# TAMUCrypto/virgo-plus

Measured on AMD Instinct MI355X. Metric: prover sec + field-ops/sec, SHA-256 circuit, 1/2/4/8 MI355X (bit-exact), higher is better.
Workload: dtype u64 (F_p^2, p=2^61-1); 1 GPU; SHA-256 1024-block circuit (SHA256_64.pws x1024, 102347776 gates, 15 layers, 2^23 input wires), GKR sumcheck + Virgo FFT/LDT commit on GPU (BASELINE configs[2]); pass_mode=sync, field_ops_per_proof=8299342697

## Files before the change

include/vpgpu.h:

```cpp
#ifndef VPGPU_H
#define VPGPU_H
#include <stdint.h>
#ifdef __cplusplus
extern "C" {
#endif

typedef struct vp_ctx vp_ctx;
typedef struct { uint64_t real, img; } vp_F;

enum {
    VP_OK = 0,
    VP_EINVAL = -1,
    VP_EHIP = -2,
    VP_ENOGPU = -3,
    VP_EASSERT = -4,
    VP_ELIMIT = -5,
    VP_EXCHANGE = 1
};

enum { VP_MUL = 0, VP_ADD, VP_SUB, VP_ANTISUB, VP_NAAB, VP_ANTINAAB, VP_INPUT, VP_MULC, VP_ADDC, VP_XOR, VP_NOT, VP_COPY };

typedef struct {
    uint64_t size;
    int32_t bit_length;
// ... 13 lines not shown
typedef struct {
    uint32_t struct_size;
    uint32_t abi;
    int32_t use_graph;
    int32_t plan_autotune;
    int32_t real_values;
    int32_t real_pairs;
    int32_t pc_tensor_pub;
    int32_t persistent_rounds;
    int32_t persistent_timeout_ms;
    int32_t poll;
    int32_t prefetch_round1;
    int32_t interactive_fast_init;
    int32_t split_cost_percent;
    int32_t debug;
    int32_t reserved[4];
} vp_options;
void vp_options_default(vp_options *opt);

int vp_create(int device, vp_ctx **out);
int vp_create_with_options(int device, const vp_options *opt, vp_ctx **out);
int vp_get_options(const vp_ctx *, vp_options *out);
int vp_tuning_get(const vp_ctx *, const char *name, int32_t *value);
int vp_test_drivers(void);
int vp_plan_tuning_get(const vp_ctx *, int32_t v[6]);
int vp_plan_tuning_set(vp_ctx *, const int32_t v[6]);
#define VP_WARM_COMMITMENT 1u
#define VP_WARM_FFT_GKR 2u
int vp_warm(vp_ctx *, uint32_t what);
void vp_destroy(vp_ctx *);
const char *vp_last_error(const vp_ctx *);
const char *vp_version(void);
int vp_checked_build(void);

int vp_circuit_upload(vp_ctx *, int n_layers, const vp_layer_desc *layers);

int vp_evaluate(vp_ctx *, const vp_F *inputs, uint64_t n_inputs);
int vp_layer_values(vp_ctx *, int layer, vp_F *out, uint64_t n);

int vp_vres(vp_ctx *, const vp_F *r_0, int r_0_size, vp_F *out);

int vp_phase1_init(vp_ctx *, int layer, const vp_F *r_liu, const vp_F *assert_random);
int vp_phase2_init(vp_ctx *, int layer, const vp_F *r_u);
int vp_liu_init(vp_ctx *, int layer, const vp_F *r_u, const vp_F *const *r_v, const vp_F *s);

int vp_round(vp_ctx *, const vp_F *previous_random, vp_F out_poly[3]);
// ... 94 lines not shown
int vp_get_resident_resumes(const vp_ctx *, uint64_t *n);
int vp_set_profiling(vp_ctx *, int level);

enum { VP_K_BETA = 0, VP_K_LIGHT, VP_K_CHUNKS, VP_K_COMBINE, VP_K_DOT, VP_K_DOTFIN, VP_K_SFGEN, VP_K_SF, VP_K_SEG, VP_K_EMIT,
       VP_K_FIXUP, VP_K_NTT_SPLIT, VP_K_NTT_LDS, VP_K_NTT_UNSPLIT, VP_K_LEAF_HASH, VP_K_MERKLE, VP_K_PC_POINTWISE, VP_K_FRI_FOLD,
       VP_K_ROUND, VP_K_NTT8_COLS, VP_K_NTT8_ROWS, VP_K_NTT_LONG_SPLIT, VP_K_NTT_LONG_MERGE, VP_K_PC_POLY_EVAL, VP_K_PC_POLY_EVAL_FIN, VP_K_PC_OPENING_DIGESTS,
       VP_K_PC_OPEN_MANY, VP_K_COUNT };
typedef struct {
    int32_t kind;
    int32_t step;
    uint32_t workgroups;
    uint32_t jobs;
    uint32_t rounds, first_round;
    uint64_t bytes;
    uint64_t work;
    double us;
} vp_launch_stat;
int vp_get_launch_stats(vp_ctx *, vp_launch_stat *out, int capacity, int *n);
const char *vp_kernel_name(int kind);

int vp_test_field(vp_ctx *, int op, const vp_F *a, const vp_F *b, vp_F *out, uint64_t n);
int vp_test_beta(vp_ctx *, const vp_F *r, int n, const vp_F *init, vp_F *out);
int vp_test_sha3(vp_ctx *, const uint8_t *in, uint8_t *out, uint64_t n);
int vp_test_fft(vp_ctx *, const vp_F *coefs, int coef_len, int order, int inverse, vp_F *out);
int vp_test_fs_draw(vp_ctx *, int op, const uint8_t state[32], const uint8_t root[32], uint64_t label, uint64_t counter, uint8_t state_out[32], vp_F *r_out);

#ifdef __cplusplus
}
#endif
#endif
```

virgo-plus_amd/__init__.py:

```python
import ctypes
import os
import shutil
import subprocess

PKG_DIR = os.path.dirname(os.path.abspath(__file__))
ROOT = os.path.dirname(PKG_DIR)
CSRC = os.path.join(PKG_DIR, "csrc")
HOST = os.path.join(PKG_DIR, "host")
LIB_GPU = os.environ.get("VP_LIBGPU") or os.path.join(CSRC, "libvpgpu.so")
LIB_GPU_CHECKED = os.path.join(ROOT, "tools", "_build", "checked", "libvpgpu.so")
LIB_GPU_TESTDRV = os.path.join(ROOT, "tools", "_build", "testdrv", "libvpgpu.so")
LIB_HOST = os.path.join(HOST, "libvphost.so")
CLI = os.path.join(HOST, "virgo_plus_run")

GPU_SRC = [os.path.join(CSRC, f) for f in ("vpgpu.hip", "vpgpu_batched.inc", "vpgpu_pc.inc", "vpgpu_pc_shard.inc", "vpgpu_pcverify.inc", "vp_kernels_pcverify.h", "vpgpu_fftgkr.inc", "vpgpu_gkrfs.inc", "vpgpu_upload.inc", "vp_kernels_fftgkr.h", "vp_kernels_gkrfs.h", "vp_kernels.h", "vp_kernels_round.h", "vp_kernels_persist.h", "vp_kernels_batch.h",
                                              "vp_kernels_plan.h", "vp_kernels_pc.h", "vp_kernels_ntt8.h", "vp_kernels_ntt_long.h", "vp_keccak_asm.h", "vp_check.h", "vp_field.h", "vp_fri_layout.h", "vp_pc_live.h", "vp_pc_corners.h")] + [
    os.path.join(ROOT, "include", "vpgpu.h")]
HOST_SRC = [os.path.join(HOST, f) for f in ("circuit.cpp", "prover.cpp", "verifier.cpp", "vphost.cpp")]
HOST_HDR = [os.path.join(HOST, f) for f in ("circuit.hpp", "prover.hpp", "verifier.hpp", "vphost.h", "field.hpp",
                                              "polynomial.hpp", "sha3.hpp", "pc_fs.hpp", "fft_gkr_fs.hpp", "gkr_fs.hpp", "fft_gkr_verify.hpp")]


def _stale(target, sources):
    if not os.path.exists(target):
# ... 65 lines not shown

_gpu = None
_host = None


def lib_gpu():
    global _gpu
    if _gpu is None:
        if not os.path.exists(LIB_GPU):
            raise RuntimeError("libvpgpu.so is not built: run __graft_entry__.build()")
        L = ctypes.CDLL(LIB_GPU, mode=ctypes.RTLD_GLOBAL)
        vp = ctypes.c_void_p
        L.vp_create.argtypes = [ctypes.c_int, ctypes.POINTER(vp)]
        L.vp_create_with_options.argtypes = [ctypes.c_int, vp, ctypes.POINTER(vp)]
        L.vp_get_options.argtypes = [vp, vp]
        L.vp_get_resident_resumes.argtypes = [vp, ctypes.POINTER(ctypes.c_uint64)]
        L.vp_set_shard_split.argtypes = [vp, ctypes.c_int]
        L.vp_set_round_shard.argtypes = [vp, ctypes.c_int, ctypes.c_int, ctypes.c_int]
        L.vp_get_round_shard.argtypes = [vp, ctypes.POINTER(ctypes.c_int), ctypes.POINTER(ctypes.c_int), ctypes.POINTER(ctypes.c_int)]
        L.vp_shard_finish.argtypes = [vp, vp, ctypes.c_uint64, vp]
        L.vp_gkr_sizes.argtypes = [vp, vp, vp]
        L.vp_options_default.argtypes = [vp]
        L.vp_tuning_get.argtypes = [vp, ctypes.c_char_p, ctypes.POINTER(ctypes.c_int32)]
        u64_ = ctypes.c_uint64
        L.vp_set_deferred.argtypes = [vp, ctypes.c_int]
        L.vp_warm.argtypes = [vp, ctypes.c_uint32]
        L.vp_flush.argtypes = [vp, ctypes.c_int]
        L.vp_pending.argtypes = [vp, ctypes.POINTER(ctypes.c_int)]
        L.vp_pc_hash_late.argtypes = [vp, ctypes.c_int]
        L.vp_phase_ms.argtypes = [vp, ctypes.POINTER(ctypes.c_double)]
        L.vp_commit_private.argtypes = [vp, vp]
        L.vp_fft_gkr_sizes.argtypes = [ctypes.c_int, vp, vp]
        L.vp_fft_gkr.argtypes = [vp, ctypes.c_int, vp, u64_, vp, u64_, vp]
        L.vp_fft_gkr_begin.argtypes = [vp, ctypes.c_int, vp, u64_]
        L.vp_fft_gkr_end.argtypes = [vp, vp, u64_, vp]
        L.vp_fft_gkr_cancel.argtypes = [vp]
        L.vp_fft_gkr_fs.argtypes = [vp, ctypes.c_int, vp, vp, u64_, vp, vp, vp]
        L.vp_options_default.restype = None
        L.vp_destroy.argtypes = [vp]
        L.vp_last_error.argtypes = [vp]
        L.vp_last_error.restype = ctypes.c_char_p
        L.vp_version.restype = ctypes.c_char_p
        L.vp_test_field.argtypes = [vp, ctypes.c_int, vp, vp, vp, ctypes.c_uint64]
        L.vp_test_beta.argtypes = [vp, vp, ctypes.c_int, vp, vp]
        L.vp_test_sha3.argtypes = [vp, vp, vp, ctypes.c_uint64]
        L.vp_test_fft.argtypes = [vp, vp, ctypes.c_int, ctypes.c_int, ctypes.c_int, vp]
# ... 649 lines not shown
        nd = ctypes.c_uint64(0)
        if lib_host().vph_gkr_fs_tape(self.h, ctypes.cast(st_in, ctypes.c_void_p), ctypes.cast(buf, ctypes.c_void_p), len(transcript), tape.ctypes.data, ctypes.byref(nd),
                                      ctypes.cast(st_out, ctypes.c_void_p)):
            raise ValueError("gkr_fs_tape: malformed transcript")
        return tape, int(nd.value), st_out.raw

    def verify_fs(self, proof):
        buf = ctypes.create_string_buffer(bytes(proof), len(proof))
        return lib_host().vph_verify_fs(self.h, ctypes.cast(buf, ctypes.c_void_p), len(proof)) == 0

    def close(self):
        if self.h:
            lib_host().vph_circuit_free(self.h)
            self.h = None


_PUBLIC_OPTIONS = ("use_graph", "plan_autotune", "real_values", "real_pairs", "pc_tensor_pub", "persistent_rounds", "persistent_timeout_ms", "poll", "prefetch_round1",
                   "interactive_fast_init", "split_cost_percent", "debug")
_TUNING_ENV = {"gkr_path": "VP_GKR_PATH", "serial": "VP_GKR_SERIAL", "fuse_init": "VP_FUSE_INIT", "fuse_min_log": "VP_FUSE_MIN_LOG", "fuse_dot": "VP_FUSE_DOT",
               "drop_y": "VP_DROP_Y", "drop_y_round1": "VP_DROP_Y1", "seg_tiny": "VP_SEG_TINY", "sf_big_log": "VP_SF_BIG_LOG", "sf3b_grid": "VP_SF3B_GRID",
               "dot_blocks": "VP_DOT_BLOCKS", "plan_align": "VP_PLAN_ALIGN", "round_fused_max": "VP_ROUND_FUSED_MAX",
               "kernel_copies": "VP_KERNEL_COPIES", "fold_branches": "VP_FOLD_BRANCHES", "fuse_combine": "VP_FUSE_COMBINE",
               "graph_explicit": "VP_GRAPH_EXPLICIT", "ntt_r8": "VP_NTT_R8", "fuse_p2": "VP_FUSE_P2", "leaf_asm": "VP_LEAF_ASM",
               "fft_gkr_batched": "VP_FFT_GKR_BATCHED", "split_vu": "VP_SPLIT_VU", "pc_live": "VP_PC_LIVE"}
VP_OPTIONS_ABI = 0x76700005


class Options(ctypes.Structure):
    _fields_ = [("struct_size", ctypes.c_uint32), ("abi", ctypes.c_uint32)] + [(n, ctypes.c_int32) for n in _PUBLIC_OPTIONS] + [("reserved", ctypes.c_int32 * 4)]

    def __init__(self, **kw):
        super().__init__()
        lib_gpu().vp_options_default(ctypes.byref(self))
        self.tuning = {}
        for k, v in kw.items():
            if k in _PUBLIC_OPTIONS:
                setattr(self, k, v)
            elif k in _TUNING_ENV:
                self.tuning[k] = v
            else:
                raise TypeError("unknown option " + k)

    def tuning_env(self):
        env = {}
        for k, v in getattr(self, "tuning", {}).items():
            if k == "gkr_path":
                v = {PATH_PLAN: "plan", PATH_LANES: "lanes", PATH_SIMPLE: "simple"}[v]
# ... 599 lines not shown
```

virgo-plus_amd/csrc/vp_kernels_pc.h:

```cpp
#pragma once
#include "vp_kernels_round.h"
#include "vp_keccak_asm.h"
#define f_mul f_mul_plain

namespace vp {

__device__ __forceinline__ F root_raw(const F *__restrict__ RT, u32 half_m , u32 e ) { return RT[e & (half_m - 1)]; }
__device__ __forceinline__ F root_fin(const F &r, u32 half_m, u32 e) {
    const bool neg = e >= half_m;
    const u64 nre = r.re ? P61 - r.re : 0, nim = r.im ? P61 - r.im : 0;
    return f_make(neg ? nre : r.re, neg ? nim : r.im);
}
__device__ __forceinline__ F root_pow(const F *__restrict__ RT, u32 half_m, u32 e) { return root_fin(root_raw(RT, half_m, e), half_m, e); }
__device__ __forceinline__ void loads_first() { __builtin_amdgcn_sched_barrier(0); }
__global__ void __launch_bounds__(VP_BLOCK)
k_root_table_step(F *RT, u32 have , F step ) {
    u32 i = blockIdx.x * blockDim.x + threadIdx.x;
    if (i < have) RT[have + i] = f_mul(RT[i], step);
}
__global__ void __launch_bounds__(VP_BLOCK) k_root_compact(const F *__restrict__ RT, u32 stride, u32 n, F *__restrict__ out) {
    const u32 k = blockIdx.x * blockDim.x + threadIdx.x;
    if (k < n) out[k] = RT[(size_t) k * stride];
}

// ... 252 lines not shown
__global__ void __launch_bounds__(VP_BLOCK) k_merkle_top_fs(MerkleArgs a, Dig *roots, Dig *state, u64 label, u64 counter, F *r_next) {
    merkle_top_body(a, roots);
    if (blockIdx.x == 0 && threadIdx.x == 0) fs_absorb_draw(state, a.tree[0] + 1, label, counter, r_next);
}
__global__ void k_fs_draw(Dig *state, const Dig *root, u64 label, u64 counter, F *r_out) {
    if (blockIdx.x == 0 && threadIdx.x == 0) fs_absorb_draw(state, root, label, counter, r_out);
}
__global__ void k_test_fs_limbs(const u64 *__restrict__ in, u64 *__restrict__ out, u32 n) {
    const u32 i = blockIdx.x * blockDim.x + threadIdx.x;
    if (i < n) out[i] = fs_limb(in[i]);
}

#ifdef VP_LEAF_STAMPS
__device__ unsigned long long g_leaf_stamps[4 * 65536];
__device__ unsigned int g_leaf_stamp_n;
#define VP_LEAF_STAMP_BEGIN const u64 st_t0 = __builtin_amdgcn_s_memtime(), st_r0 = __builtin_amdgcn_s_memrealtime();
#define VP_LEAF_STAMP_END(tag) if (threadIdx.x == 0) { const u64 st_t1 = __builtin_amdgcn_s_memtime(), st_r1 = __builtin_amdgcn_s_memrealtime(); \
        const u32 sl = atomicAdd(&g_leaf_stamp_n, 1u) & 65535u; g_leaf_stamps[4 * sl] = st_t0; g_leaf_stamps[4 * sl + 1] = st_r0; g_leaf_stamps[4 * sl + 2] = st_t1; \
        g_leaf_stamps[4 * sl + 3] = (st_r1 << 1) | (tag); }
#else
#define VP_LEAF_STAMP_BEGIN
#define VP_LEAF_STAMP_END(tag)
#endif
template <bool MASK> __global__ void __launch_bounds__(VP_LEAF_ASM_THREADS) k_leaf_hash(FriLeafArgs a) {
    VP_LEAF_STAMP_BEGIN
    const u32 total = a.leaf_start[a.n];
    const u32 g = blockIdx.x * blockDim.x + threadIdx.x, gc = g < total ? g : total - 1;
    int j = 0;
    while (j + 1 < a.n && gc >= a.leaf_start[j + 1]) ++j;
    const u32 t = gc - a.leaf_start[j], N = a.N[j];
    const F *cw = a.cw[j];
    const bool last = N == 1;
    const u32 halfN = last ? 16u : N >> 1;
    const u32 p = last ? t : t % halfN, b = last ? 0u : t / halfN;
    const F *x = cw + (size_t) b * N + p;
    if constexpr (MASK) {
        const F *m = a.mask[j] + (size_t) b * N + p;
        vp_leaf_chain_mask_asm(x, x + halfN, 32u * N * 16u, 64u, m, m + halfN, a.leaves[j] + (last ? t : 32 * p + b), g < total ? 1u : 0u);
    } else
        vp_leaf_chain_asm(x, x + halfN, 32u * N * 16u, 64u, a.leaves[j] + (last ? t : 32 * p + b), g < total ? 1u : 0u);
    VP_LEAF_STAMP_END(a.n > 1 ? 1u : 0u)
}

__global__ void k_test_sha3(const u64 *__restrict__ in, u64 *__restrict__ out, u32 n) {
    u32 i = blockIdx.x * blockDim.x + threadIdx.x;
    if (i >= n) return;
    Dig h; h.w[0] = in[8 * i + 4]; h.w[1] = in[8 * i + 5]; h.w[2] = in[8 * i + 6]; h.w[3] = in[8 * i + 7];
    Dig d = hhash64(in[8 * i], in[8 * i + 1], in[8 * i + 2], in[8 * i + 3], h);
    out[4 * i] = d.w[0]; out[4 * i + 1] = d.w[1]; out[4 * i + 2] = d.w[2]; out[4 * i + 3] = d.w[3];
}

}

namespace vp {

__global__ void __launch_bounds__(VP_BLOCK)
k_pc_products(const F *__restrict__ lcw, const F *__restrict__ qcw, u32 N, F *__restrict__ P, u32 n_slices, const F *__restrict__ q0,
              const F *__restrict__ qscal) {
    const u32 t = blockIdx.x * blockDim.x + threadIdx.x;
    if (t >= 2 * n_slices * N) return;
    const u32 a = t % N, r = t / N, i = r >> 1, b = (r & 1) ? 16 : 0;
    const size_t src = ((size_t) i * 32 + b) * N + a;
    const F q = q0 ? f_mul(qscal[i], q0[(size_t) b * N + a]) : qcw[src];
    P[t] = f_mul(lcw[src], q);
// ... 485 lines not shown
```

virgo-plus_amd/csrc/vpgpu.hip:

```cpp
#include <hip/hip_runtime.h>

#include <algorithm>
#include <chrono>
#include <cstdio>
#include <cstring>
#include <deque>
#include <functional>
#include <map>
#include <mutex>
#include <set>
#include <atomic>
#include <string>
#include <thread>
#include <vector>

#include "../../include/vpgpu.h"
#include "vp_kernels.h"
#include "vp_fri_layout.h"
#include "vp_pc_live.h"
#include "vp_pc_corners.h"

using namespace vp;

static_assert(sizeof(vp_F) == sizeof(F), "vp_F layout");
// ... 107 lines not shown
    int32_t drop_y;
    int32_t drop_y_round1;
    int32_t real_values;
    int32_t seg_tiny;
    int32_t sf_big_log;
    int32_t sf3b_grid;
    int32_t dot_blocks;
    int32_t plan_align;
    int32_t round_fused_max;
    int32_t persistent_rounds, poll, debug, prefetch_round1, split_cost_percent;
    int32_t kernel_copies;
    int32_t fold_branches;
    int32_t fuse_combine;
    int32_t plan_autotune, pc_tensor_pub, persistent_timeout_ms;
    int32_t graph_explicit;
    int32_t ntt_r8;
    int32_t interactive_fast_init;
    int32_t fuse_p2;
    int32_t leaf_asm;
    int32_t real_pairs;
    int32_t fft_gkr_batched;
    int32_t split_vu;
    int32_t pc_live;
};

struct vp_ctx {
    int device = 0;
    hipStream_t stream = nullptr;
    std::string err = "";
    int n_layers = 0, max_bl = 0;
    std::vector<LayerDev> L;
    F **d_vals = nullptr;
    unsigned long long **d_valsr = nullptr;
    F *beta_g = nullptr, *beta_u = nullptr, *bf = nullptr, *bs = nullptr, *liu_half = nullptr;
    u32 half_cap = 0;
    F *tab[2][3] = {{nullptr, nullptr, nullptr}, {nullptr, nullptr, nullptr}};
    u32 cap = 0;
    F *partials = nullptr;
    unsigned int *round_arrivals = nullptr;
    F *small = nullptr;
    F *chunk_part = nullptr; u32 chunk_cap = 0;
    F *d_tape = nullptr; u64 n_tape = 0;
    F *d_tr = nullptr; u64 n_tr = 0;
    F *h_pin = nullptr;
    unsigned long long *h_seq = nullptr, seq = 0;
    TailMail *h_req = nullptr; TailReply *h_rep = nullptr; std::atomic<bool> tail_active{false}; unsigned long long tail_seq = 0; int tail_enabled = 1;
// ... 51 lines not shown
    int hash_late = 0;
    unsigned pc_unhashed = 0;
    uint8_t *late_root[2] = {nullptr, nullptr};

    PcShard *pcs = nullptr;
    FgkState *fgk = nullptr;
    VpComm *cm = nullptr;
    F *part2 = nullptr;
    int simple_path = 0, serial = 0;
    Lane lane0; Lane *ln = nullptr;
    std::vector<Lane> lanes;
    std::vector<hipStream_t> lane_streams; std::vector<hipEvent_t> lane_events; hipEvent_t ev_fork = nullptr;
    F *pred_r = nullptr, *pred_pool = nullptr, *pred_part = nullptr, *pred_out = nullptr; BetaJob *pred_jobs = nullptr; u32 pred_bpj = 1;
    DotJob *pred_dot = nullptr; BlkMap *pred_map = nullptr;
    PlanRec *rec = nullptr;
    DotJob rec_dot{};
    SfGenJob rec_gen{};
    int fuse_init = 1;
    Plan *plan = nullptr; int plan_path = 1;
    std::recursive_mutex mu;
    bool plan_tuned = false;
    bool plan_tune_cached = false;
    int leaf_attr_done = 0;
    uint32_t opt_pinned = 0;
    hipGraphExec_t gkr_graph = nullptr; int use_graph = 1; bool graph_failed = false; u64 graph_launches = 0, graph_rounds = 0;
    int shard_rank = 0, shard_world = 1;
    int split_lw = 0, split_min_log = 11;
    struct SplitTab { int j, bl; u32 slot0; };
    struct SplitChain { u64 poly_pos = 0, claims_pos = 0, r_off = 0; int rounds = 0, has_a = 1, n_tab = 0, small_owner = 0; std::vector<SplitTab> tabs; };
    std::vector<SplitChain> split;
    F *d_trs = nullptr; u64 n_exp = 0;
    F *tr_base() const { return (split_lw > 0 && d_trs) ? d_trs : d_tr; }
    std::vector<int> chain_owner;
    std::vector<double> chain_cost;
    bool drop_round1 = false;
    std::vector<FixJob> rec_fix;
    bool owned(int chain) const { return shard_world <= 1 || chain_owner.empty() || chain_owner[chain] == shard_rank; }
    bool vu_supplied = false; float vu_pre_ms = 0; u64 vu_tape_tag = 0;
    RoundShard *rsh = nullptr;
    bool sc_open = false;

    F *zero() const { return small; }
    F *one() const { return small + 1; }
    F *add_term() const { return small + 2; }
    F *Vu() const { return small + 3; }
    F *coef() const { return small + 4; }
// ... 667 lines not shown
    return 0;
#endif
}
const char *vp_version(void) { return "vpgpu 0.1 (gfx950)"; }
const char *vp_last_error(const vp_ctx *ctx) { return ctx ? ctx->err.c_str() : "null context"; }

static void opt_defaults(VpOpt *o) {
    memset(o, 0, sizeof *o);
    o->gkr_path = VP_PATH_PLAN; o->use_graph = 1; o->serial = 0; o->fuse_init = 1; o->fuse_min_log = 0; o->fuse_dot = 0;
    o->drop_y = 1; o->drop_y_round1 = 0; o->real_values = 1; o->seg_tiny = 1; o->sf_big_log = 14;
    o->sf3b_grid = 512; o->dot_blocks = 1024; o->plan_align = 0; o->round_fused_max = 512;
    o->persistent_rounds = 1; o->poll = 1; o->debug = 0; o->prefetch_round1 = 1; o->split_cost_percent = 50; o->kernel_copies = 1; o->fold_branches = 1; o->fuse_combine = 2; o->plan_autotune = 1;
    o->pc_tensor_pub = 1;
    o->persistent_timeout_ms = 10000;
    o->graph_explicit = 0;
    o->ntt_r8 = 1;
    o->interactive_fast_init = 1;
    o->fuse_p2 = 1;
    o->leaf_asm = 1;
    o->real_pairs = 1;
    o->fft_gkr_batched = 1;
    o->split_vu = 1;
    o->pc_live = 1;
}
static void opt_to_public(const VpOpt &o, vp_options *p) {
    memset(p, 0, sizeof *p);
    p->struct_size = (uint32_t) sizeof *p; p->abi = VP_OPTIONS_ABI;
    p->use_graph = o.use_graph; p->plan_autotune = o.plan_autotune; p->real_values = o.real_values; p->real_pairs = o.real_pairs; p->pc_tensor_pub = o.pc_tensor_pub;
    p->persistent_rounds = o.persistent_rounds; p->persistent_timeout_ms = o.persistent_timeout_ms; p->poll = o.poll; p->prefetch_round1 = o.prefetch_round1;
    p->interactive_fast_init = o.interactive_fast_init; p->split_cost_percent = o.split_cost_percent; p->debug = o.debug;
}
void vp_options_default(vp_options *p) {
    if (!p) return;
    VpOpt o; opt_defaults(&o);
    opt_to_public(o, p);
}
int vp_test_drivers(void) {
#ifdef VP_TEST_DRIVERS
    return 1;
#else
    return 0;
#endif
}
struct OptName { const char *name; int32_t VpOpt::*field; };
static const OptName g_opt_names[] = {
    {"gkr_path", &VpOpt::gkr_path}, {"use_graph", &VpOpt::use_graph}, {"serial", &VpOpt::serial}, {"fuse_init", &VpOpt::fuse_init}, {"fuse_min_log", &VpOpt::fuse_min_log},
    {"fuse_dot", &VpOpt::fuse_dot}, {"drop_y", &VpOpt::drop_y}, {"drop_y_round1", &VpOpt::drop_y_round1}, {"real_values", &VpOpt::real_values}, {"seg_tiny", &VpOpt::seg_tiny},
    {"sf_big_log", &VpOpt::sf_big_log}, {"sf3b_grid", &VpOpt::sf3b_grid}, {"dot_blocks", &VpOpt::dot_blocks}, {"plan_align", &VpOpt::plan_align},
    {"round_fused_max", &VpOpt::round_fused_max}, {"persistent_rounds", &VpOpt::persistent_rounds}, {"poll", &VpOpt::poll}, {"debug", &VpOpt::debug},
    {"prefetch_round1", &VpOpt::prefetch_round1}, {"split_cost_percent", &VpOpt::split_cost_percent}, {"kernel_copies", &VpOpt::kernel_copies},
    {"fold_branches", &VpOpt::fold_branches}, {"fuse_combine", &VpOpt::fuse_combine}, {"plan_autotune", &VpOpt::plan_autotune},
    {"pc_tensor_pub", &VpOpt::pc_tensor_pub}, {"persistent_timeout_ms", &VpOpt::persistent_timeout_ms}, {"graph_explicit", &VpOpt::graph_explicit}, {"ntt_r8", &VpOpt::ntt_r8},
    {"interactive_fast_init", &VpOpt::interactive_fast_init}, {"fuse_p2", &VpOpt::fuse_p2}, {"leaf_asm", &VpOpt::leaf_asm},
    {"real_pairs", &VpOpt::real_pairs}, {"fft_gkr_batched", &VpOpt::fft_gkr_batched}, {"split_vu", &VpOpt::split_vu}, {"pc_live", &VpOpt::pc_live}};
int vp_tuning_get(const vp_ctx *ctx, const char *name, int32_t *value) {
    if (!ctx || !name || !value) return VP_EINVAL;
    for (const OptName &n : g_opt_names) if (!strcmp(n.name, name)) { *value = ctx->opt.*(n.field); return VP_OK; }
    return VP_EINVAL;
}
static int resolve_options(VpOpt *o, const vp_options *user, uint32_t *pinned) {
    opt_defaults(o);
    if (user) {
        if (user->struct_size != sizeof(vp_options) || user->abi != VP_OPTIONS_ABI) return VP_EINVAL;
        o->use_graph = user->use_graph; o->plan_autotune = user->plan_autotune; o->real_values = user->real_values; o->real_pairs = user->real_pairs;
        o->pc_tensor_pub = user->pc_tensor_pub; o->persistent_rounds = user->persistent_rounds; o->persistent_timeout_ms = user->persistent_timeout_ms;
        o->poll = user->poll; o->prefetch_round1 = user->prefetch_round1; o->interactive_fast_init = user->interactive_fast_init;
        o->split_cost_percent = user->split_cost_percent; o->debug = user->debug;
    }
    auto flag = [](const char *name, int32_t &v) { const char *e = getenv(name); if (e && (e[0] == '0' || e[0] == '1')) v = e[0] - '0'; };
    auto num = [](const char *name, int32_t &v) { const char *e = getenv(name); if (e && *e) v = atoi(e); };
    if (const char *p = getenv("VP_GKR_PATH"))
        o->gkr_path = !strcmp(p, "lanes") ? VP_PATH_LANES : !strcmp(p, "simple") ? VP_PATH_SIMPLE : VP_PATH_PLAN;
#ifndef VP_TEST_DRIVERS
    if (o->gkr_path != VP_PATH_PLAN) return VP_EINVAL;
#endif
    if (const char *p = getenv("VP_PLAN_ALIGN")) o->plan_align = !strcmp(p, "left") ? 1 : !strcmp(p, "right") ? 2 : 0;
    flag("VP_GKR_GRAPH", o->use_graph); flag("VP_GKR_SERIAL", o->serial); flag("VP_FUSE_INIT", o->fuse_init); flag("VP_FUSE_DOT", o->fuse_dot);
    flag("VP_DROP_Y", o->drop_y); flag("VP_DROP_Y1", o->drop_y_round1); flag("VP_REAL_V", o->real_values);
    flag("VP_SEG_TINY", o->seg_tiny); flag("VP_PERSIST", o->persistent_rounds);
    flag("VP_POLL", o->poll); flag("VP_PREFETCH_R1", o->prefetch_round1);
    num("VP_FUSE_MIN_LOG", o->fuse_min_log); num("VP_SF_BIG_LOG", o->sf_big_log);
    num("VP_SF3B_GRID", o->sf3b_grid); num("VP_DOT_BLOCKS", o->dot_blocks);
    num("VP_ROUND_FUSED_MAX", o->round_fused_max);
    num("VP_SPLIT_COST_PERCENT", o->split_cost_percent);
    flag("VP_KERNEL_COPIES", o->kernel_copies);
    flag("VP_FOLD_BRANCHES", o->fold_branches);
    flag("VP_NTT_R8", o->ntt_r8);
    flag("VP_FAST_INIT", o->interactive_fast_init);
    flag("VP_FUSE_P2", o->fuse_p2);
    flag("VP_LEAF_ASM", o->leaf_asm);
    flag("VP_REAL_PAIRS", o->real_pairs);
    flag("VP_FFT_GKR_BATCHED", o->fft_gkr_batched);
    flag("VP_SPLIT_VU", o->split_vu);
    flag("VP_PC_LIVE", o->pc_live);
    flag("VP_PC_TENSOR", o->pc_tensor_pub);
    num("VP_PERSIST_TIMEOUT_MS", o->persistent_timeout_ms);
    num("VP_GRAPH_EXPLICIT", o->graph_explicit);
    num("VP_FUSE_COMBINE", o->fuse_combine);
    flag("VP_PLAN_AUTOTUNE", o->plan_autotune);
    if (getenv("VP_DEBUG")) o->debug |= 1;
    if (getenv("VP_DEBUG_UPLOAD")) o->debug |= 2;
    o->dot_blocks = std::max(1, o->dot_blocks); o->sf3b_grid = std::max(1, o->sf3b_grid);
    VpOpt d; opt_defaults(&d);
    *pinned = (o->fuse_combine != d.fuse_combine ? 1u : 0u) | (o->fold_branches != d.fold_branches ? 2u : 0u) | (o->plan_align != d.plan_align ? 4u : 0u) |
              (o->fuse_min_log != d.fuse_min_log ? 8u : 0u) | (o->sf3b_grid != d.sf3b_grid ? 16u : 0u) | (o->graph_explicit != d.graph_explicit ? 32u : 0u);
    return VP_OK;
}

int vp_plan_tuning_get(const vp_ctx *ctx, int32_t v[6]) {
    if (!ctx || !v) return VP_EINVAL;
    v[0] = ctx->opt.fuse_combine; v[1] = ctx->opt.fold_branches; v[2] = ctx->opt.plan_align; v[3] = ctx->opt.fuse_min_log; v[4] = ctx->opt.sf3b_grid; v[5] = ctx->opt.graph_explicit;
    return VP_OK;
}
int vp_plan_tuning_set(vp_ctx *ctx, const int32_t v[6]) {
    if (!ctx || !v) return VP_EINVAL;
    if (v[0] < 0 || v[0] > 2 || v[1] < 0 || v[1] > 1 || v[2] < 0 || v[2] > 2 || v[3] < 0 || v[3] > 30 || v[4] < 1 || v[4] > 4096 || v[5] < 0 || v[5] > 3) return VP_EINVAL;
    VP_ENTER(ctx);
// ... 13 lines not shown
struct RandKeep {
    char priv[128]; char *caller;
    RandKeep() { g_rand_mu.lock(); memset(priv, 0, sizeof priv); caller = initstate(1u, priv, sizeof priv); }
    ~RandKeep() { if (caller) setstate(caller); g_rand_mu.unlock(); }
};

int vp_create_with_options(int device, const vp_options *user, vp_ctx **out) {
    if (!out) return VP_EINVAL;
    *out = nullptr;
    RandKeep keep_callers_random_stream;
    int n = 0;
    if (hipGetDeviceCount(&n) != hipSuccess || n <= 0 || device < 0 || device >= n) return VP_ENOGPU;
    if (hipSetDevice(device) != hipSuccess) return VP_ENOGPU;
    vp_ctx *ctx = new vp_ctx();
    ctx->device = device;
    if (resolve_options(&ctx->opt, user, &ctx->opt_pinned) != VP_OK) { delete ctx; return VP_EINVAL; }
    if (const char *pcf = getenv("VP_PLAN_CACHE")) ctx->plan_cache_path = pcf;
    if (hipStreamCreateWithFlags(&ctx->stream, hipStreamNonBlocking) != hipSuccess) { delete ctx; return VP_EHIP; }
    if (hipHostMalloc((void **) &ctx->h_pin, (4 + VP_MAX_TAB) * sizeof(F), hipHostMallocDefault) != hipSuccess) {
        delete ctx; return VP_EHIP;
    }
    if (hipHostMalloc((void **) &ctx->h_seq, 64, hipHostMallocDefault) != hipSuccess) { delete ctx; return VP_EHIP; }
    *ctx->h_seq = 0;
    if (hipHostMalloc((void **) &ctx->h_req, sizeof(TailMail), hipHostMallocDefault) != hipSuccess ||
        hipHostMalloc((void **) &ctx->h_rep, sizeof(TailReply), hipHostMallocDefault) != hipSuccess) { delete ctx; return VP_EHIP; }
    if (hipHostMalloc((void **) &ctx->h_aux, sizeof(TailAux), hipHostMallocDefault) != hipSuccess) { delete ctx; return VP_EHIP; }
    if (hipHostMalloc((void **) &ctx->h_stage, 4096 * sizeof(F), hipHostMallocDefault) != hipSuccess) { delete ctx; return VP_EHIP; }
    memset(ctx->h_req, 0, sizeof(TailMail)); memset(ctx->h_rep, 0, sizeof(TailReply)); memset(ctx->h_aux, 0, sizeof(TailAux));
    (void) hipFuncSetAttribute(reinterpret_cast<const void *>(k_phase), hipFuncAttributeMaxDynamicSharedMemorySize, 3 * 2 * VP_PH_PMAX * (int) sizeof(F));
    ctx->poll = ctx->opt.poll; ctx->tail_enabled = ctx->opt.persistent_rounds;
    hipEventCreate(&ctx->ev0); hipEventCreate(&ctx->ev1);
    (void) hipFuncSetAttribute(reinterpret_cast<const void *>(k_emit_multi), hipFuncAttributeMaxDynamicSharedMemorySize, 160 * 1024 - 256);
    (void) hipFuncSetAttribute(reinterpret_cast<const void *>(k_emit), hipFuncAttributeMaxDynamicSharedMemorySize, 160 * 1024 - 256);
    (void) hipFuncSetAttribute(reinterpret_cast<const void *>(k_ntt_lds), hipFuncAttributeMaxDynamicSharedMemorySize, 160 * 1024 - 256);
    (void) hipFuncSetAttribute(reinterpret_cast<const void *>(k_ntt8_cols<false>), hipFuncAttributeMaxDynamicSharedMemorySize, 80 * 1024);
    (void) hipFuncSetAttribute(reinterpret_cast<const void *>(k_ntt8_cols<true>), hipFuncAttributeMaxDynamicSharedMemorySize, 80 * 1024);
    (void) hipFuncSetAttribute(reinterpret_cast<const void *>(k_ntt8_rows<false>), hipFuncAttributeMaxDynamicSharedMemorySize, 80 * 1024);
    (void) hipFuncSetAttribute(reinterpret_cast<const void *>(k_ntt8_rows<true>), hipFuncAttributeMaxDynamicSharedMemorySize, 80 * 1024);
    { std::lock_guard<std::mutex> lk(g_ctx_mu); g_ctxs.push_back(ctx); }
    *out = ctx;
    return VP_OK;
}

static void free_plan(vp_ctx *ctx);
void vp_free_shard_state(vp_ctx *ctx);
void vp_free_comm(vp_ctx *ctx);
// ... 1 lines not shown

static void rs_free(vp_ctx *ctx);
void vp_destroy(vp_ctx *ctx) {
    if (!ctx) return;
    if (tl_entry_depth == 0) vp_suspend_others(ctx);
    { std::lock_guard<std::mutex> lk(g_ctx_mu); g_ctxs.erase(std::remove(g_ctxs.begin(), g_ctxs.end(), ctx), g_ctxs.end()); }
    { std::lock_guard<std::recursive_mutex> lo(ctx->mu); }
    (void) hipSetDevice(ctx->device);
    if (ctx->tail_active) (void) tail_quit(ctx);
    (void) hipStreamSynchronize(ctx->stream);
    (void) pc_hash_outstanding(ctx, 3u);
    vp_free_shard_state(ctx);
    rs_free(ctx);
    vp_free_comm(ctx);
    vp_free_fgk(ctx);
    if (ctx->gkr_graph) (void) hipGraphExecDestroy(ctx->gkr_graph);
    free_plan(ctx);
    free_all(ctx);
    for (auto &e : ctx->ev_pool) { (void) hipEventDestroy(e.a); (void) hipEventDestroy(e.b); }
    if (ctx->ev0) (void) hipEventDestroy(ctx->ev0);
    if (ctx->ev1) (void) hipEventDestroy(ctx->ev1);
    if (ctx->h_pin) (void) hipHostFree(ctx->h_pin);
    if (ctx->h_seq) (void) hipHostFree(ctx->h_seq);
    if (ctx->h_req) (void) hipHostFree(ctx->h_req);
    if (ctx->h_rep) (void) hipHostFree(ctx->h_rep);
    if (ctx->h_aux) (void) hipHostFree(ctx->h_aux);
    if (ctx->h_stage) (void) hipHostFree(ctx->h_stage);
    if (ctx->h_io) (void) hipHostFree(ctx->h_io);
    if (ctx->h_ring) (void) hipHostFree(ctx->h_ring);
    if (ctx->h_pub) (void) hipHostFree(ctx->h_pub);
    if (ctx->h_many) (void) hipHostFree(ctx->h_many);
    for (auto &p : ctx->pending) { (void) hipEventDestroy(p.a); (void) hipEventDestroy(p.b); }
    for (auto e : ctx->ev_spare) (void) hipEventDestroy(e);
    for (auto st : ctx->lane_streams) (void) hipStreamDestroy(st);
    for (auto ev : ctx->lane_events) (void) hipEventDestroy(ev);
    if (ctx->ev_fork) (void) hipEventDestroy(ctx->ev_fork);
    (void) hipStreamDestroy(ctx->stream);
    delete ctx;
}

int vp_circuit_upload(vp_ctx *ctx, int n_layers, const vp_layer_desc *ld) {
    if (!ctx || !ld || n_layers < 2) return VP_EINVAL;
    if (n_layers > VP_MAX_TAB) { ctx->err = "too many layers"; return VP_ELIMIT; }
    RandKeep keep_callers_random_stream;
    VP_ENTER(ctx);
    VPCHK(pc_hash_outstanding(ctx, 3u));
// ... 904 lines not shown
```

virgo-plus_amd/csrc/vpgpu_pc.inc:

```
namespace {

constexpr int PC_MAX_LN = 13;
#ifndef VP_NTT_SPLIT_LOG
#define VP_NTT_SPLIT_LOG 12
#endif
constexpr int PC_SPLIT_LN = VP_NTT_SPLIT_LOG;

#define PC_PROF_IF(on, kind, grid, jobs, bytes, work, ...)                                               \
    do {                                                                                                  \
        const int sl_ = (on) ? prof_begin(ctx, ctx->stream, (kind), (u32) (grid), (u32) (jobs), (u64) (bytes), (u64) (work)) : -1; \
        __VA_ARGS__;                                                                      \
        prof_end(ctx, ctx->stream, sl_);                                                                  \
    } while (0)
#define PC_PROF(kind, grid, jobs, bytes, work, ...) PC_PROF_IF(true, kind, grid, jobs, bytes, work, __VA_ARGS__)

F host_pow(F x, unsigned __int128 e) { F r = f_one(); while (e) { if (e & 1) r = f_mul(r, x); x = f_mul(x, x); e >>= 1; } return r; }
F host_root_of_unity(int log_order) {
    F r = f_make(2147483648ull, 1033321771269002680ull);
    for (int i = 0; i < 62 - log_order; ++i) r = f_mul(r, r);
    return r;
}
F host_inv_real(u64 x) { return host_pow(f_make(x, 0), (unsigned __int128) P61 - 2); }

int pc_root_fill(vp_ctx *ctx, F *rt, int lm) {
// ... 265 lines not shown
    }
    return VP_OK;
}

static inline u32 pc_leaf_wg(const vp_ctx *ctx, u64 n_leaves) {
#ifdef VP_CHECKED
    (void) ctx; (void) n_leaves; return 0;
#else
    if (!ctx->opt.leaf_asm) return 0;
    return n_leaves >= (1u << 18) ? 1024u : n_leaves >= (1u << 17) ? 512u : 0u;
#endif
}
static inline size_t pc_leaf_lds(u32 wg) { return wg == 1024 ? 0 : 96 * 1024; }
static inline int pc_leaf_prepare(vp_ctx *ctx) {
    if (ctx->leaf_attr_done) return ctx->leaf_attr_done > 0 ? VP_OK : VP_EHIP;
    hipError_t err = hipFuncSetAttribute((const void *) k_leaf_hash<false>, hipFuncAttributeMaxDynamicSharedMemorySize, 96 * 1024);
    if (err == hipSuccess) err = hipFuncSetAttribute((const void *) k_leaf_hash<true>, hipFuncAttributeMaxDynamicSharedMemorySize, 96 * 1024);
    ctx->leaf_attr_done = err == hipSuccess ? 1 : -1;
    if (err != hipSuccess) { ctx->err = "hipFuncSetAttribute (leaf hash)"; return VP_EHIP; }
    return VP_OK;
}
static int pc_hash_leaves(vp_ctx *ctx, FriLeafArgs &la, bool profiled) {
    if (la.n < 1) return VP_OK;
    u32 blocks = 0, leaves = 0;
    int n_masked = 0;
    for (int q = 0; q < la.n; ++q) {
        const u32 nl = la.N[q] >= 2 ? 16 * la.N[q] : 16u;
        la.blk_start[q] = blocks; la.leaf_start[q] = leaves;
        blocks += nblk(nl); leaves += nl;
        if (la.mask[q]) ++n_masked;
    }
    la.blk_start[la.n] = blocks; la.leaf_start[la.n] = leaves;
    if (n_masked && n_masked != la.n) { ctx->err = "internal: leaf-hash entries with and without a mask slice in one launch"; return VP_EINVAL; }
    u32 wg = pc_leaf_wg(ctx, leaves);
    if (wg && pc_leaf_prepare(ctx) != VP_OK) wg = 0;
    const void *kernel = !wg ? (const void *) k_leaf_hash_c : n_masked ? (const void *) k_leaf_hash<true> : (const void *) k_leaf_hash<false>;
    void *args[] = {&la};
    PC_PROF_IF(profiled, VP_K_LEAF_HASH, blocks, la.n, (u64) leaves * (64 * 32 + 32), (u64) leaves * 65,
               (void) hipLaunchKernel(kernel, dim3(wg ? (leaves + wg - 1) / wg : blocks), dim3(wg ? wg : VP_BLOCK), args, wg ? pc_leaf_lds(wg) : 0, ctx->stream));
    return VP_OK;
}

struct PcFsTop { Dig *state; u64 label, counter; F *r_next; };
static int pc_merkle_trees(vp_ctx *ctx, MerkleArgs &ma, Dig *d_roots, int levels = -1, const PcFsTop *fs = nullptr) {
    for (int h = 0; levels < 0 || h < levels; ++h) {
        MerkleArgs lv{}; u32 b = 0; u64 hs = 0;
        for (int q = 0; q < ma.n; ++q) {
            const u32 c = ma.count[q] >> 1;
            if (levels < 0 && c <= 512) continue;
            lv.tree[lv.n] = ma.tree[q]; lv.count[lv.n] = c; lv.blk_start[lv.n] = b; b += nblk(c); hs += c; ++lv.n;
            ma.count[q] = c;
        }
        if (!lv.n) break;
        lv.blk_start[lv.n] = b;
        PC_PROF(VP_K_MERKLE, b, lv.n, 96ull * hs, hs, hipLaunchKernelGGL(k_merkle_level, dim3(b), dim3(VP_BLOCK), 0, ctx->stream, lv));
    }
    if (levels >= 0) return VP_OK;
    u64 hs = 0;
    for (int q = 0; q < ma.n; ++q) hs += ma.count[q] - 1;
    if (fs) {
        if (ma.n != 1) { ctx->err = "internal: the drawing tree top takes one tree"; return VP_EINVAL; }
        const int sl_ = prof_begin(ctx, ctx->stream, VP_K_MERKLE, 1, 1, 96ull * hs + 3 * 64, hs + 3, 1, (u32) (fs->label - 1));
// ... 990 lines not shown
}

int vp_commit_stats(vp_ctx *ctx, double *commit_ms) {
    if (!ctx || !commit_ms) return VP_EINVAL;
    *commit_ms = ctx->commit_ms;
    return VP_OK;
}

int vp_test_sha3(vp_ctx *ctx, const uint8_t *in, uint8_t *out, uint64_t n) {
    if (!ctx || !in || !out) return VP_EINVAL;
    if (!n) return VP_OK;
    VP_ENTER(ctx);
    u64 *di = nullptr, *dout = nullptr;
    HIPCHK(hipMalloc((void **) &di, n * 64));
    HIPCHK(hipMalloc((void **) &dout, n * 32));
    HIPCHK(hipMemcpy(di, in, n * 64, hipMemcpyHostToDevice));
    hipLaunchKernelGGL(k_test_sha3, dim3((unsigned) ((n + 255) / 256)), dim3(256), 0, ctx->stream, di, dout, (u32) n);
    int rc = check_stream(ctx);
    if (rc == VP_OK && hipMemcpy(out, dout, n * 32, hipMemcpyDeviceToHost) != hipSuccess) rc = VP_EHIP;
    (void) hipFree(di); (void) hipFree(dout);
    return rc;
}

#ifdef VP_LEAF_STAMPS
int vp_debug_leaf_stamps(vp_ctx *ctx, uint64_t *out, unsigned cap, unsigned *n) {
    if (!ctx || !out || !n) return VP_EINVAL;
    VP_ENTER(ctx);
    HIPCHK(hipStreamSynchronize(ctx->stream));
    unsigned cnt = 0;
    HIPCHK(hipMemcpyFromSymbol(&cnt, HIP_SYMBOL(g_leaf_stamp_n), sizeof cnt));
    *n = std::min(std::min(cnt, 65536u), cap);
    if (*n) HIPCHK(hipMemcpyFromSymbol(out, HIP_SYMBOL(g_leaf_stamps), (size_t) *n * 32));
    cnt = 0;
    HIPCHK(hipMemcpyToSymbol(HIP_SYMBOL(g_leaf_stamp_n), &cnt, sizeof cnt));
    return VP_OK;
}
int vp_debug_leaf_only(vp_ctx *ctx, int reps) {
    if (!ctx || !ctx->pc_private_done || ctx->pcs) return VP_EINVAL;
    VP_ENTER(ctx);
    const int n = ctx->L[0].bl;
    FriLeafArgs la{};
    la.cw[0] = ctx->pc_cw; la.leaves[0] = ctx->pc_tree + (1u << (n - 2)); la.N[0] = 1u << (n - 6); la.n = 1;
    for (int i = 0; i < reps; ++i) VPCHK(pc_hash_leaves(ctx, la, false));
    return check_stream(ctx);
}
#endif
// ... 37 lines not shown
```

Measured before the change: 167.3 billion field-ops/s.

## Hash FRI leaves with persistent walker blocks claiming tiles via atomic counter

The leaf-hash kernel now launches at most one workgroup per CU (configurable) instead of one per tile. Each workgroup loops over tiles, claiming the next one through a global atomic counter whose value is passed to the other threads by double-buffered shared memory. A small close kernel checks that every tile was hashed, resets the counter, and flags a host-visible error otherwise. The aim is to cut workgroup launch and tail overhead and balance load across CUs. In exchange it adds an atomic and a barrier per tile, an extra kernel launch, and may lose latency hiding if a single resident workgroup per CU is not enough.

```diff
diff --git a/include/vpgpu.h b/include/vpgpu.h
--- a/include/vpgpu.h
+++ b/include/vpgpu.h
@@ -59,6 +59,7 @@
 int vp_create_with_options(int device, const vp_options *opt, vp_ctx **out);
 int vp_get_options(const vp_ctx *, vp_options *out);
 int vp_tuning_get(const vp_ctx *, const char *name, int32_t *value);
+int vp_tuning_set(vp_ctx *, const char *name, int32_t value);
 int vp_test_drivers(void);
 int vp_plan_tuning_get(const vp_ctx *, int32_t v[6]);
 int vp_plan_tuning_set(vp_ctx *, const int32_t v[6]);
@@ -199,6 +200,9 @@
 int vp_test_field(vp_ctx *, int op, const vp_F *a, const vp_F *b, vp_F *out, uint64_t n);
 int vp_test_beta(vp_ctx *, const vp_F *r, int n, const vp_F *init, vp_F *out);
 int vp_test_sha3(vp_ctx *, const uint8_t *in, uint8_t *out, uint64_t n);
+int vp_test_pc_tree(vp_ctx *, int oracle, uint8_t *out, uint64_t cap, uint64_t *n_bytes);
+int vp_test_pc_poison_trees(vp_ctx *);
+int vp_test_leaf_claim(vp_ctx *, int64_t set_counter, uint32_t out[3]);
 int vp_test_fft(vp_ctx *, const vp_F *coefs, int coef_len, int order, int inverse, vp_F *out);
 int vp_test_fs_draw(vp_ctx *, int op, const uint8_t state[32], const uint8_t root[32], uint64_t label, uint64_t counter, uint8_t state_out[32], vp_F *r_out);
 
diff --git a/virgo-plus_amd/__init__.py b/virgo-plus_amd/__init__.py
--- a/virgo-plus_amd/__init__.py
+++ b/virgo-plus_amd/__init__.py
@@ -111,6 +111,7 @@
         L.vp_gkr_sizes.argtypes = [vp, vp, vp]
         L.vp_options_default.argtypes = [vp]
         L.vp_tuning_get.argtypes = [vp, ctypes.c_char_p, ctypes.POINTER(ctypes.c_int32)]
+        L.vp_tuning_set.argtypes = [vp, ctypes.c_char_p, ctypes.c_int32]
         u64_ = ctypes.c_uint64
         L.vp_set_deferred.argtypes = [vp, ctypes.c_int]
         L.vp_warm.argtypes = [vp, ctypes.c_uint32]
@@ -806,7 +807,8 @@
                "dot_blocks": "VP_DOT_BLOCKS", "plan_align": "VP_PLAN_ALIGN", "round_fused_max": "VP_ROUND_FUSED_MAX",
                "kernel_copies": "VP_KERNEL_COPIES", "fold_branches": "VP_FOLD_BRANCHES", "fuse_combine": "VP_FUSE_COMBINE",
                "graph_explicit": "VP_GRAPH_EXPLICIT", "ntt_r8": "VP_NTT_R8", "fuse_p2": "VP_FUSE_P2", "leaf_asm": "VP_LEAF_ASM",
-               "fft_gkr_batched": "VP_FFT_GKR_BATCHED", "split_vu": "VP_SPLIT_VU", "pc_live": "VP_PC_LIVE"}
+               "fft_gkr_batched": "VP_FFT_GKR_BATCHED", "split_vu": "VP_SPLIT_VU", "pc_live": "VP_PC_LIVE",
+               "leaf_walkers": "VP_LEAF_WALKERS", "leaf_claim": "VP_LEAF_CLAIM"}
 VP_OPTIONS_ABI = 0x76700005
 
 
diff --git a/virgo-plus_amd/csrc/vp_kernels_pc.h b/virgo-plus_amd/csrc/vp_kernels_pc.h
--- a/virgo-plus_amd/csrc/vp_kernels_pc.h
+++ b/virgo-plus_amd/csrc/vp_kernels_pc.h
@@ -298,24 +298,48 @@
 #define VP_LEAF_STAMP_BEGIN
 #define VP_LEAF_STAMP_END(tag)
 #endif
-template <bool MASK> __global__ void __launch_bounds__(VP_LEAF_ASM_THREADS) k_leaf_hash(FriLeafArgs a) {
-    VP_LEAF_STAMP_BEGIN
-    const u32 total = a.leaf_start[a.n];
-    const u32 g = blockIdx.x * blockDim.x + threadIdx.x, gc = g < total ? g : total - 1;
-    int j = 0;
-    while (j + 1 < a.n && gc >= a.leaf_start[j + 1]) ++j;
-    const u32 t = gc - a.leaf_start[j], N = a.N[j];
-    const F *cw = a.cw[j];
-    const bool last = N == 1;
-    const u32 halfN = last ? 16u : N >> 1;
-    const u32 p = last ? t : t % halfN, b = last ? 0u : t / halfN;
-    const F *x = cw + (size_t) b * N + p;
-    if constexpr (MASK) {
-        const F *m = a.mask[j] + (size_t) b * N + p;
-        vp_leaf_chain_mask_asm(x, x + halfN, 32u * N * 16u, 64u, m, m + halfN, a.leaves[j] + (last ? t : 32 * p + b), g < total ? 1u : 0u);
-    } else
-        vp_leaf_chain_asm(x, x + halfN, 32u * N * 16u, 64u, a.leaves[j] + (last ? t : 32 * p + b), g < total ? 1u : 0u);
-    VP_LEAF_STAMP_END(a.n > 1 ? 1u : 0u)
+template <bool MASK> __global__ void __launch_bounds__(VP_LEAF_ASM_THREADS) k_leaf_hash(FriLeafArgs a, u32 *claim) {
+    __shared__ u32 s_tile[2];
+    const u32 total = a.leaf_start[a.n], tiles = (total + blockDim.x - 1) / blockDim.x;
+    int j0 = 0;
+    u32 slot = 0, hashed = 0;
+    for (u32 tile = blockIdx.x; tile < tiles;) {
+        VP_LEAF_STAMP_BEGIN
+        u32 nxt = 0;
+        if (claim && threadIdx.x == 0) nxt = atomicAdd(claim, 1u);
+        const u32 g0 = tile * blockDim.x;
+        while (j0 + 1 < a.n && g0 >= a.leaf_start[j0 + 1]) ++j0;
+        const u32 g = g0 + threadIdx.x, gc = g < total ? g : total - 1;
+        int j = j0;
+        while (j + 1 < a.n && gc >= a.leaf_start[j + 1]) ++j;
+        const u32 t = gc - a.leaf_start[j], N = a.N[j];
+        const F *cw = a.cw[j];
+        const bool last = N == 1;
+        const u32 halfN = last ? 16u : N >> 1;
+        const u32 p = last ? t : t % halfN, b = last ? 0u : t / halfN;
+        const F *x = cw + (size_t) b * N + p;
+        if (claim && threadIdx.x == 0) s_tile[slot] = gridDim.x + nxt;
+        if constexpr (MASK) {
+            const F *m = a.mask[j] + (size_t) b * N + p;
+            vp_leaf_chain_mask_asm(x, x + halfN, 32u * N * 16u, 64u, m, m + halfN, a.leaves[j] + (last ? t : 32 * p + b), g < total ? 1u : 0u);
+        } else
+            vp_leaf_chain_asm(x, x + halfN, 32u * N * 16u, 64u, a.leaves[j] + (last ? t : 32 * p + b), g < total ? 1u : 0u);
+        VP_LEAF_STAMP_END(a.n > 1 ? 1u : 0u)
+        if (claim) {
+            __syncthreads();
+            tile = __builtin_amdgcn_readfirstlane(s_tile[slot]);
+            slot ^= 1u; ++hashed;
+        } else
+            tile += gridDim.x;
+    }
+    if (claim && threadIdx.x == 0) atomicAdd(claim + 1, hashed);
+}
+
+__global__ void k_leaf_claim_close(u32 *claim, u32 tiles, volatile u32 *host_dirty) {
+    if (blockIdx.x == 0 && threadIdx.x == 0) {
+        if (claim[1] != tiles) *host_dirty = 1u;
+        claim[0] = 0u; claim[1] = 0u;
+    }
 }
 
 __global__ void k_test_sha3(const u64 *__restrict__ in, u64 *__restrict__ out, u32 n) {
diff --git a/virgo-plus_amd/csrc/vpgpu.hip b/virgo-plus_amd/csrc/vpgpu.hip
--- a/virgo-plus_amd/csrc/vpgpu.hip
+++ b/virgo-plus_amd/csrc/vpgpu.hip
@@ -153,6 +153,8 @@
     int32_t fft_gkr_batched;
     int32_t split_vu;
     int32_t pc_live;
+    int32_t leaf_walkers;
+    int32_t leaf_claim;
 };
 
 struct vp_ctx {
@@ -250,6 +252,9 @@
     bool plan_tuned = false;
     bool plan_tune_cached = false;
     int leaf_attr_done = 0;
+    int n_cu = 0;
+    u32 *leaf_claim = nullptr;
+    u32 *h_leaf_dirty = nullptr;
     uint32_t opt_pinned = 0;
     hipGraphExec_t gkr_graph = nullptr; int use_graph = 1; bool graph_failed = false; u64 graph_launches = 0, graph_rounds = 0;
     int shard_rank = 0, shard_world = 1;
@@ -963,6 +968,8 @@
     o->fft_gkr_batched = 1;
     o->split_vu = 1;
     o->pc_live = 1;
+    o->leaf_walkers = -1;
+    o->leaf_claim = 1;
 }
 static void opt_to_public(const VpOpt &o, vp_options *p) {
     memset(p, 0, sizeof *p);
@@ -993,10 +1000,18 @@
     {"fold_branches", &VpOpt::fold_branches}, {"fuse_combine", &VpOpt::fuse_combine}, {"plan_autotune", &VpOpt::plan_autotune},
     {"pc_tensor_pub", &VpOpt::pc_tensor_pub}, {"persistent_timeout_ms", &VpOpt::persistent_timeout_ms}, {"graph_explicit", &VpOpt::graph_explicit}, {"ntt_r8", &VpOpt::ntt_r8},
     {"interactive_fast_init", &VpOpt::interactive_fast_init}, {"fuse_p2", &VpOpt::fuse_p2}, {"leaf_asm", &VpOpt::leaf_asm},
-    {"real_pairs", &VpOpt::real_pairs}, {"fft_gkr_batched", &VpOpt::fft_gkr_batched}, {"split_vu", &VpOpt::split_vu}, {"pc_live", &VpOpt::pc_live}};
+    {"real_pairs", &VpOpt::real_pairs}, {"fft_gkr_batched", &VpOpt::fft_gkr_batched}, {"split_vu", &VpOpt::split_vu}, {"pc_live", &VpOpt::pc_live},
+    {"leaf_walkers", &VpOpt::leaf_walkers}, {"leaf_claim", &VpOpt::leaf_claim}};
 int vp_tuning_get(const vp_ctx *ctx, const char *name, int32_t *value) {
     if (!ctx || !name || !value) return VP_EINVAL;
     for (const OptName &n : g_opt_names) if (!strcmp(n.name, name)) { *value = ctx->opt.*(n.field); return VP_OK; }
+    return VP_EINVAL;
+}
+int vp_tuning_set(vp_ctx *ctx, const char *name, int32_t value) {
+    if (!ctx || !name) return VP_EINVAL;
+    VP_ENTER(ctx);
+    if (!strcmp(name, "leaf_walkers") && value >= -1 && value <= 65535) { ctx->opt.leaf_walkers = value; return VP_OK; }
+    if (!strcmp(name, "leaf_claim") && (value == 0 || value == 1)) { ctx->opt.leaf_claim = value; return VP_OK; }
     return VP_EINVAL;
 }
 static int resolve_options(VpOpt *o, const vp_options *user, uint32_t *pinned) {
@@ -1034,6 +1049,7 @@
     flag("VP_FFT_GKR_BATCHED", o->fft_gkr_batched);
     flag("VP_SPLIT_VU", o->split_vu);
     flag("VP_PC_LIVE", o->pc_live);
+    num("VP_LEAF_WALKERS", o->leaf_walkers); flag("VP_LEAF_CLAIM", o->leaf_claim);
     flag("VP_PC_TENSOR", o->pc_tensor_pub);
     num("VP_PERSIST_TIMEOUT_MS", o->persistent_timeout_ms);
     num("VP_GRAPH_EXPLICIT", o->graph_explicit);
@@ -1093,6 +1109,10 @@
     }
     if (hipHostMalloc((void **) &ctx->h_seq, 64, hipHostMallocDefault) != hipSuccess) { delete ctx; return VP_EHIP; }
     *ctx->h_seq = 0;
+    if (hipDeviceGetAttribute(&ctx->n_cu, hipDeviceAttributeMultiprocessorCount, device) != hipSuccess || ctx->n_cu < 1) { delete ctx; return VP_EHIP; }
+    if (hipMalloc((void **) &ctx->leaf_claim, 64) != hipSuccess || hipMemset(ctx->leaf_claim, 0, 64) != hipSuccess) { delete ctx; return VP_EHIP; }
+    if (hipHostMalloc((void **) &ctx->h_leaf_dirty, 64, hipHostMallocDefault) != hipSuccess) { delete ctx; return VP_EHIP; }
+    *ctx->h_leaf_dirty = 0;
     if (hipHostMalloc((void **) &ctx->h_req, sizeof(TailMail), hipHostMallocDefault) != hipSuccess ||
         hipHostMalloc((void **) &ctx->h_rep, sizeof(TailReply), hipHostMallocDefault) != hipSuccess) { delete ctx; return VP_EHIP; }
     if (hipHostMalloc((void **) &ctx->h_aux, sizeof(TailAux), hipHostMallocDefault) != hipSuccess) { delete ctx; return VP_EHIP; }
@@ -1140,6 +1160,8 @@
     if (ctx->ev1) (void) hipEventDestroy(ctx->ev1);
     if (ctx->h_pin) (void) hipHostFree(ctx->h_pin);
     if (ctx->h_seq) (void) hipHostFree(ctx->h_seq);
+    if (ctx->leaf_claim) (void) hipFree(ctx->leaf_claim);
+    if (ctx->h_leaf_dirty) (void) hipHostFree(ctx->h_leaf_dirty);
     if (ctx->h_req) (void) hipHostFree(ctx->h_req);
     if (ctx->h_rep) (void) hipHostFree(ctx->h_rep);
     if (ctx->h_aux) (void) hipHostFree(ctx->h_aux);
diff --git a/virgo-plus_amd/csrc/vpgpu_pc.inc b/virgo-plus_amd/csrc/vpgpu_pc.inc
--- a/virgo-plus_amd/csrc/vpgpu_pc.inc
+++ b/virgo-plus_amd/csrc/vpgpu_pc.inc
@@ -311,6 +311,7 @@
 }
 static int pc_hash_leaves(vp_ctx *ctx, FriLeafArgs &la, bool profiled) {
     if (la.n < 1) return VP_OK;
+    if (*ctx->h_leaf_dirty) { ctx->err = "leaf hash: the claim counter was not zero at an earlier launch, or its walk went wrong (tiles were skipped)"; return VP_EHIP; }
     u32 blocks = 0, leaves = 0;
     int n_masked = 0;
     for (int q = 0; q < la.n; ++q) {
@@ -324,9 +325,17 @@
     u32 wg = pc_leaf_wg(ctx, leaves);
     if (wg && pc_leaf_prepare(ctx) != VP_OK) wg = 0;
     const void *kernel = !wg ? (const void *) k_leaf_hash_c : n_masked ? (const void *) k_leaf_hash<true> : (const void *) k_leaf_hash<false>;
-    void *args[] = {&la};
+    const u32 tiles = wg ? (leaves + wg - 1) / wg : blocks;
+    u32 grid = tiles;
+    u32 *claim = nullptr;
+    if (const u32 walkers = ctx->opt.leaf_walkers < 0 ? (u32) ctx->n_cu : (u32) ctx->opt.leaf_walkers; wg && walkers) {
+        grid = std::min(grid, walkers);
+        if (ctx->opt.leaf_claim) claim = ctx->leaf_claim;
+    }
+    void *args[] = {&la, &claim};
     PC_PROF_IF(profiled, VP_K_LEAF_HASH, blocks, la.n, (u64) leaves * (64 * 32 + 32), (u64) leaves * 65,
-               (void) hipLaunchKernel(kernel, dim3(wg ? (leaves + wg - 1) / wg : blocks), dim3(wg ? wg : VP_BLOCK), args, wg ? pc_leaf_lds(wg) : 0, ctx->stream));
+               (void) hipLaunchKernel(kernel, dim3(grid), dim3(wg ? wg : VP_BLOCK), args, wg ? pc_leaf_lds(wg) : 0, ctx->stream));
+    if (claim) hipLaunchKernelGGL(k_leaf_claim_close, dim3(1), dim3(64), 0, ctx->stream, claim, tiles, (volatile u32 *) ctx->h_leaf_dirty);
     return VP_OK;
 }
 
@@ -1363,6 +1372,39 @@
     return rc;
 }
 
+int vp_test_leaf_claim(vp_ctx *ctx, int64_t set_counter, uint32_t out[3]) {
+    if (!ctx || !out) return VP_EINVAL;
+    CtxLock lk(ctx, true);
+    HIPCHK(hipSetDevice(ctx->device));
+    HIPCHK(hipStreamSynchronize(ctx->stream));
+    if (set_counter >= 0) { const u32 v = (u32) set_counter; HIPCHK(hipMemcpy(ctx->leaf_claim, &v, 4, hipMemcpyHostToDevice)); }
+    HIPCHK(hipMemcpy(out, ctx->leaf_claim, 8, hipMemcpyDeviceToHost));
+    out[2] = *ctx->h_leaf_dirty;
+    return VP_OK;
+}
+int vp_test_pc_poison_trees(vp_ctx *ctx) {
+    if (!ctx || ctx->L.empty() || ctx->pcs) return VP_EINVAL;
+    VP_ENTER(ctx);
+    VPCHK(pc_hash_outstanding(ctx, 3u));
+    HIPCHK(hipStreamSynchronize(ctx->stream));
+    const size_t bytes = ((size_t) 1 << (ctx->L[0].bl - 1)) * sizeof(Dig);
+    for (Dig *t : {ctx->pc_tree, ctx->pc_tree_h, ctx->pc_fri_tree}) if (t) HIPCHK(hipMemset(t, 0xA5, bytes));
+    return VP_OK;
+}
+int vp_test_pc_tree(vp_ctx *ctx, int oracle, uint8_t *out, uint64_t cap, uint64_t *n_bytes) {
+    if (!ctx || !n_bytes) return VP_EINVAL;
+    VP_ENTER(ctx);
+    if (ctx->pcs) return VP_EINVAL;
+    PcOpenDesc d;
+    VPCHK(pc_open_desc(ctx, oracle, &d));
+    *n_bytes = (2ull * d.n_leaves - 1) * sizeof(Dig);
+    if (!out) return VP_OK;
+    if (cap < *n_bytes) return VP_EINVAL;
+    HIPCHK(hipStreamSynchronize(ctx->stream));
+    HIPCHK(hipMemcpy(out, d.tree + 1, *n_bytes, hipMemcpyDeviceToHost));
+    return VP_OK;
+}
+
 #ifdef VP_LEAF_STAMPS
 int vp_debug_leaf_stamps(vp_ctx *ctx, uint64_t *out, unsigned cap, unsigned *n) {
     if (!ctx || !out || !n) return VP_EINVAL;
```

Result: no change. 166.2 billion field-ops/s, median of 3 (-0.7%).
